# Tzq2doc/distributed_learning_simulator

Hardware: AMD Instinct MI355X
Metric: FL rounds/sec (FedAvg, 100 clients, ResNet-18, CIFAR-10-shaped) (higher is better)
Workload: dtype fp32; 1 GPU; fedavg_resnet18; model=ResNet18, algo=fed_avg, clients=100, local_epochs=5, global_batch=6400, per_client_batch=64, parallelism=client-dp1, backend=hip

## Files before the change

csrc/conv_halo.hip:

```cpp
#include "dls.h"
#include "epilogue_f32.h"
#include "gemm_common.h"

namespace {

typedef __attribute__((address_space(3))) void lds_void;

__device__ __forceinline__ void hdma16(__amdgpu_buffer_rsrc_t r, unsigned char* lds, uint32_t off) {
  __builtin_amdgcn_raw_ptr_buffer_load_lds(r, (lds_void*)lds, 16, off, 0, 0, 0);
}

template <int N>
__device__ __forceinline__ void hwait_vm() {
  static_assert(N >= 0 && N < 64, "vmcnt range");
  __builtin_amdgcn_s_waitcnt((N & 15) | ((N >> 4) << 14) | (7 << 4) | (15 << 8));
}

template <int IMG, int TH, int TW, int BN, int WM, int WN, bool BKM, int MINW, int HB, int NBS, int BNM = 0,
          int TPS = 1>
__global__ void __launch_bounds__(WM* WN * 64) __attribute__((amdgpu_waves_per_eu(MINW * WM * WN / 4)))
conv_halo_kernel(ConvNTParams p) {
  constexpr bool BNF = BNM != 0, DENSE = BNM == 2;
  static_assert((HB == 2 && NBS == 3) || (HB == 1 && (NBS == 2 || NBS == 3)), "pipeline shape");
  static_assert(TPS == 1 || (HB == 1 && TPS == 2 && NBS == 2), "taps per step");
// ... 212 lines not shown
        const bool real = BI * NW == NBI || i * NW + wid < NBI;
        if (TPS > 1 && !real) continue;
        unsigned char* d = real ? Bs + (i * NW + wid) * 1024 : smem + SCR;
        hdma16(br, d, ok ? off : OOB_OFF);
        hdma16(br, real ? d + B_PL : d, ok ? off + b_lo : OOB_OFF);
      }
    }
  };

  f32x16 acc[TM][TN];
#pragma unroll
  for (int i = 0; i < TM; ++i)
#pragma unroll
    for (int j = 0; j < TN; ++j) acc[i][j] = f32x16{};

  const int wm0 = (wid / WN) * (TM * 32), wn0 = (wid % WN) * (TN * 32);
  const int g = lane >> 4, q = (lane >> 2) & 3, pp = lane & 3, h = lane >> 5;
  int hbase[TM], hkey[TM];
#pragma unroll
  for (int i = 0; i < TM; ++i) {
    const int pix = wm0 + i * 32 + (lane & 31);
    const int img = pix / (TH * TW), rr = pix - img * (TH * TW);
    const int th = rr / TW, tw = rr - th * TW;
    hbase[i] = img * HH2 * PITCH + th * PITCH + tw;
    hkey[i] = (img * HH2 + th) * KC;
  }
  const int rsw = (lane >> 2) & 3;
  auto compute = [&](int hb, int slot, int shift, int dh) {
    const unsigned char* Hs = smem + H_OFF + hb * 2 * H_PL;
    const unsigned char* Bs = smem + B_OFF + slot * 2 * B_PL;
#pragma unroll
    for (int ks = 0; ks < 2; ++ks) {
      bf16x8 ah[TM], al[TM], bh[TN], bl[TN];
#pragma unroll
      for (int i = 0; i < TM; ++i) {
        const int hr = hbase[i] + shift;
        const unsigned char* a = Hs + hr * 64 + (((ks * 2 + h) ^ (((hr >> 2) + hkey[i] + dh * KC) & 3)) << 4);
        ah[i] = *reinterpret_cast<const bf16x8*>(a);
        al[i] = *reinterpret_cast<const bf16x8*>(a + H_PL);
      }
#pragma unroll
      for (int j = 0; j < TN; ++j) {
        if constexpr (!BKM) {
          const unsigned char* b = Bs + (wn0 + j * 32 + (lane & 31)) * 64 + (((ks * 2 + h) ^ rsw) << 4);
          bh[j] = *reinterpret_cast<const bf16x8*>(b);
          bl[j] = *reinterpret_cast<const bf16x8*>(b + B_PL);
        } else {
          const int kr = ks * 16 + 8 * h + q;
          const int f = SS > 1 ? (kr / SD) & (SS - 1) : 0;
          const int col = (wn0 + j * 32 + 16 * (g & 1) + 4 * pp) ^ (f << 5);
          const bf16_t* b0p = reinterpret_cast<const bf16_t*>(Bs) + kr * BN + col;
          bh[j] = tr_frag(b0p, b0p + 4 * BN);
          bl[j] = tr_frag(b0p + B_PL / 2, b0p + B_PL / 2 + 4 * BN);
        }
      }
#pragma unroll
      for (int i = 0; i < TM; ++i)
#pragma unroll
        for (int j = 0; j < TN; ++j) {
          acc[i][j] = __builtin_amdgcn_mfma_f32_32x32x16_bf16(al[i], bh[j], acc[i][j], 0, 0, 0);
          acc[i][j] = __builtin_amdgcn_mfma_f32_32x32x16_bf16(ah[i], bl[j], acc[i][j], 0, 0, 0);
          acc[i][j] = __builtin_amdgcn_mfma_f32_32x32x16_bf16(ah[i], bh[j], acc[i][j], 0, 0, 0);
        }
    }
  };

  if constexpr (COEF_C > 0) {
    for (int i = threadIdx.x; i < 2 * p.C; i += NW * 64) coef_s[i] = bcoef[i];
    __syncthreads();
  }
  issue_halo(0, 0);
  issue_w(0, 0);
  if constexpr (NBS == 3) issue_w(1, 1);
  if constexpr (TPS > 1) {
    int c = 0, j = 0;
    for (int s = 0; s < nsteps; ++s) {
      if (j == 0 && c > 0) {
        __builtin_amdgcn_s_barrier();
        issue_halo(c, 0);
        hwait_vm<0>();
      } else {
        hwait_vm<TPS * GB*(NBS - 2)>();
      }
      __builtin_amdgcn_s_barrier();
      issue_w(s + NBS - 1, (s + NBS - 1) % NBS);
#pragma unroll
      for (int u = 0; u < TPS; ++u) {
        const int tap = j * TPS + u;
        if (tap < 9) {
          const int dh = tap / 3;
          compute(0, (s % NBS) * TPS + u, dh * PITCH + (tap - dh * 3), dh);
        }
      }
      if (++j == SPC) {
        j = 0;
        ++c;
      }
    }
  } else {
  int c = 0, tap = 0;
  for (int s = 0; s < nsteps; ++s) {
    if constexpr (HB == 2) {
      if (tap == 1 || tap == 2)
        hwait_vm<GB + GH>();
      else
        hwait_vm<GB>();
    } else {
      if (tap == 0 && c > 0) {
        __builtin_amdgcn_s_barrier();
        issue_halo(c, 0);
        hwait_vm<0>();
      } else {
        hwait_vm<GB*(NBS - 2)>();
      }
    }
    __builtin_amdgcn_s_barrier();
    issue_w(s + NBS - 1, (s + NBS - 1) % NBS);
    if constexpr (HB == 2)
      if (tap == 0) issue_halo(c + 1, (c + 1) & 1);
    const int dh = tap / 3;
    compute(HB == 2 ? (c & 1) : 0, s % NBS, dh * PITCH + (tap - dh * 3), dh);
    if (++tap == 9) {
      tap = 0;
      ++c;
    }
  }
  }
  hwait_vm<0>();

  nt_f32_epilogue<TM, TN, NW, (TM * TN <= 2 ? 2 : -1), false>(p, acc, smem, client, m0, n0, wm0, wn0, wid, lane);
}

template <int IMG, int TH, int TW, int BN, int WM, int WN, int HB, int NBS, int TPS = 1, int MINW = 1>
void launch_halo(const ConvNTParams& p, int K, hipStream_t s) {
  const int tilesM = IMG == 1 ? p.B * (p.OH / TH) : p.B / IMG;
  const int grid = K * tilesM * cdiv(p.N, BN);
  if (p.b_kmajor)
    hipLaunchKernelGGL((conv_halo_kernel<IMG, TH, TW, BN, WM, WN, true, MINW, HB, NBS, 0, TPS>), dim3(grid),
                       dim3(WM * WN * 64), 0, s, p);
  else
    hipLaunchKernelGGL((conv_halo_kernel<IMG, TH, TW, BN, WM, WN, false, MINW, HB, NBS, 0, TPS>), dim3(grid),
                       dim3(WM * WN * 64), 0, s, p);
}

template <int IMG, int TH, int TW, int BN, int WM, int WN, int NBS, int BNM = 1, int TPS = 1, int MINW = 1>
void launch_halo_bnf(const ConvNTParams& p, int K, hipStream_t s) {
  const int tilesM = IMG == 1 ? p.B * (p.OH / TH) : p.B / IMG;
  const int grid = K * tilesM * cdiv(p.N, BN);
  hipLaunchKernelGGL((conv_halo_kernel<IMG, TH, TW, BN, WM, WN, false, MINW, 1, NBS, BNM, TPS>), dim3(grid),
                     dim3(WM * WN * 64), 0, s, p);
}


int g_halo_mode = -1;
int g_halo_variant = -1;

}

void conv_halo_set_mode(int m) { g_halo_mode = m; }
void conv_halo_set_variant(int v) { g_halo_variant = v; }

static int halo_config(const ConvNTParams& p) {
  if (p.KH != 3 || p.KW != 3 || p.stride != 1 || p.pad != 1 || p.pad_w != 1 || p.dil != 1) return -1;
  const bool dense = p.bn_x != nullptr && p.bn_c > 0;
  if (p.OH != p.H || p.OW != p.W || p.out_s > 1 || p.C % 32 || p.N % (dense ? 4 : 8) || p.ldx % 8 || p.R != 9 * p.C)
    return -1;
  if ((p.x_lo == 0 && p.bn_x == nullptr) || p.wsplit == nullptr) return -1;
  if (p.bn_x != nullptr && (p.b_kmajor || (!dense && p.ldx != p.C))) return -1;
  if (p.bn_x != nullptr && p.C > (dense ? (p.OW == 8 ? 1 << 30 : 512) : (p.OW == 32 ? 128 : p.OW == 8 ? 256 : 1 << 30)))
    return -1;
  if (dense) {
    if (p.N > 32 || p.bn_c % 4 || p.bn_c > p.C || p.bn_c > p.ldx || (p.bn_y && p.bn_ldy % 4)) return -1;
    if (p.bn_mask && (!p.bn_y || p.bn_ldy % 8 || p.bn_c % 8)) return -1;
    if (p.OW == 32 && p.OH % 8 == 0) return 4;
    if (p.OW == 16 && p.OH == 16) return 5;
    if (p.OW == 8 && p.OH == 8 && p.B % 4 == 0) return 6;
    return -1;
  }
  if (p.OW == 32 && p.OH % 8 == 0 && p.N <= 64) return 0;
  if (p.OW == 16 && p.OH == 16) return 1;
  if (p.OW == 8 && p.OH == 8 && p.B % 2 == 0) return 2;
  if (p.OW == 4 && p.OH == 4 && p.B % 8 == 0 && g_halo_mode == 1) return 3;
  return -1;
}

bool conv_halo(const ConvNTParams& p, int K, hipStream_t s) {
  if (g_halo_mode == 0 || p.yp) return false;
  const int cfg = halo_config(p);
  if (cfg < 0) return false;
  const long ab = (p.x_lo + (long)p.B * p.H * p.W * p.ldx) * 2;
  const long wb = (p.ws_plane + (p.b_kmajor ? (long)p.C * p.wKH * p.wKW * p.N : (long)p.N * p.R)) * 2;
  if (ab >= (long)OOB_OFF || wb >= (long)OOB_OFF) return false;
  if (p.bn_x != nullptr) {
    if (g_halo_variant >= 0 || cfg == 3) return false;
    switch (cfg) {
      case 0: launch_halo_bnf<1, 8, 32, 64, 4, 2, 2, 1, 2, 2>(p, K, s); break;
      case 1: launch_halo_bnf<1, 16, 16, 128, 4, 2, 2>(p, K, s); break;
      case 2: launch_halo_bnf<2, 8, 8, 128, 4, 2, 2>(p, K, s); break;
      case 4: launch_halo_bnf<1, 8, 32, 32, 4, 1, 3, 2>(p, K, s); break;
      case 5: launch_halo_bnf<1, 16, 16, 32, 4, 1, 3, 2>(p, K, s); break;
      case 6: launch_halo_bnf<4, 8, 8, 32, 4, 1, 3, 2>(p, K, s); break;
      default: return false;
    }
    return true;
  }
  const int v = g_halo_variant >= 0 ? g_halo_variant : (cfg == 2 ? 2 : 1);
  if (cfg > 3) return false;
  if (cfg == 0 && (v == 1 || v == 3)) {
    launch_halo<1, 8, 32, 64, 4, 2, 1, 2, 2>(p, K, s);
    return true;
  }
  if (v > 2) return false;
  switch (cfg * 3 + v) {
    case 0: launch_halo<1, 8, 32, 64, 4, 1, 2, 3>(p, K, s); break;
    case 2: launch_halo<1, 8, 32, 64, 4, 2, 2, 3>(p, K, s); break;
    case 3: launch_halo<1, 16, 16, 128, 4, 2, 2, 3>(p, K, s); break;
    case 4: launch_halo<1, 16, 16, 128, 4, 2, 1, 2>(p, K, s); break;
    case 5: launch_halo<1, 16, 16, 128, 4, 2, 1, 3>(p, K, s); break;
    case 6: launch_halo<2, 8, 8, 128, 2, 2, 2, 3>(p, K, s); break;
    case 7: launch_halo<2, 8, 8, 128, 4, 2, 1, 3>(p, K, s); break;
    case 8: launch_halo<2, 8, 8, 128, 4, 2, 1, 2>(p, K, s); break;
    case 9: launch_halo<8, 4, 4, 128, 2, 2, 2, 3>(p, K, s); break;
    case 10: launch_halo<8, 4, 4, 128, 4, 2, 1, 3>(p, K, s); break;
    case 11: launch_halo<8, 4, 4, 128, 4, 2, 1, 2>(p, K, s); break;
    default: return false;
  }
  return true;
}

bool conv_halo_bn_supported(int B, int H, int W, int C, int N) {
  ConvNTParams p{};
  p.bn_x = reinterpret_cast<const float*>(16);
  p.wsplit = reinterpret_cast<const bf16_t*>(16);
  p.B = B; p.H = H; p.W = W; p.C = C; p.OH = H; p.OW = W; p.KH = 3; p.KW = 3;
  p.stride = 1; p.pad = 1; p.pad_w = 1; p.dil = 1; p.N = N; p.R = 9 * C; p.ldx = C; p.out_s = 1;
  const int cfg = halo_config(p);
  return g_halo_mode != 0 && g_halo_variant < 0 && cfg >= 0 && cfg != 3 && (long)B * H * W * C * 4 < (1L << 31);
}

static ConvNTParams halo_bn_params(const float* x, long x_cs, int ldx, const float* coef, int relu,
                                   const int* valid_rows, const bf16_t* wsplit, long ws_cs, long ws_plane, int rep,
                                   float* y, long y_cs, int ldy, int B, int H, int W, int C, int N, float* stats,
                                   const int* stats_valid) {
  ConvNTParams p{};
  p.f32 = 1;
  p.bn_x = x;
  p.bn_x_cs = x_cs;
  p.bn_coef = coef;
  p.bn_relu = relu;
  p.bn_valid = valid_rows;
  p.wsplit = wsplit;
  p.ws_cs = ws_cs;
  p.ws_plane = ws_plane;
  p.rep = rep;
  p.y = reinterpret_cast<bf16_t*>(y);
  p.y_cs = y_cs;
  p.B = B; p.H = H; p.W = W; p.C = C; p.OH = H; p.OW = W; p.KH = 3; p.KW = 3;
  p.stride = 1; p.pad = 1; p.pad_w = 1; p.dil = 1;
  p.M = B * H * W; p.N = N; p.R = 9 * C;
  p.wKH = 3; p.wKW = 3; p.kh_off = 2; p.kw_off = 2; p.kh_step = 1; p.kw_step = 1;
  p.out_s = 1;
  p.ldx = ldx; p.ldy = ldy;
  p.fd_ohw = make_fastdiv((uint32_t)(H * W));
  p.fd_ow = make_fastdiv((uint32_t)W);
  p.fd_kwc = make_fastdiv((uint32_t)(3 * C));
  p.fd_c = make_fastdiv((uint32_t)C);
  p.stats = stats;
  p.stats_valid = stats_valid;
  return p;
}

bool conv_halo_bn_fwd(const float* x, long x_cs, const float* coef, int relu, const int* valid_rows,
                      const bf16_t* wsplit, long ws_cs, long ws_plane, int rep, float* y, long y_cs, int K, int B,
                      int H, int W, int C, int N, float* stats, const int* stats_valid, hipStream_t s,
                      bf16_t* yp, uint8_t* mask) {
  ConvNTParams p = halo_bn_params(x, x_cs, C, coef, relu, valid_rows, wsplit, ws_cs, ws_plane, rep, y, y_cs, N, B, H,
                                  W, C, N, stats, stats_valid);
  p.bn_yp = yp;
  p.bn_mask = mask;
  if (stats && stats_valid && !yp && native_option(g_opt_halo_skip, "DLS_SKIP_INVALID", 1)) {
    p.skip_valid = stats_valid;
    p.skip_mul = H * W;
  }
  const long wb = (ws_plane + (long)N * p.R) * 2;
  if (wb >= (long)OOB_OFF || (long)p.M * C * 4 >= (1L << 31)) return false;
  return conv_halo(p, K, s);
}

bool conv_halo_bn_dense_supported(int B, int H, int W, int C, int N) {
  ConvNTParams p{};
  p.bn_x = reinterpret_cast<const float*>(16);
  p.wsplit = reinterpret_cast<const bf16_t*>(16);
  p.bn_c = 4;
  p.B = B; p.H = H; p.W = W; p.C = C; p.OH = H; p.OW = W; p.KH = 3; p.KW = 3;
  p.stride = 1; p.pad = 1; p.pad_w = 1; p.dil = 1; p.N = N; p.R = 9 * C; p.ldx = C; p.out_s = 1;
  return g_halo_mode != 0 && g_halo_variant < 0 && halo_config(p) >= 4;
}

bool conv_halo_bn_dense_fwd(const float* x, long x_cs, int ldx, int creal, const float* coef, int relu,
                            const int* valid_rows, const bf16_t* wsplit, long ws_cs, long ws_plane, int rep, float* y,
                            long y_cs, int ldy, int K, int B, int H, int W, int C, int N, float* stats,
                            const int* stats_valid, float* ny, long ny_cs, int ldny, uint8_t* mask, hipStream_t s) {
  ConvNTParams p = halo_bn_params(x, x_cs, ldx, coef, relu, valid_rows, wsplit, ws_cs, ws_plane, rep, y, y_cs, ldy, B,
                                  H, W, C, N, stats, stats_valid);
  p.bn_c = creal;
  p.bn_y = ny;
  p.bn_y_cs = ny_cs;
  p.bn_ldy = ldny;
  p.bn_mask = mask;
  const long wb = (ws_plane + (long)N * p.R) * 2;
  if (wb >= (long)OOB_OFF || (long)p.M * ldx * 4 >= (1L << 31)) return false;
  if (halo_config(p) < 4) return false;
  return conv_halo(p, K, s);
}
```

csrc/dls.h:

```cpp
#pragma once
#include <hip/hip_runtime.h>
#include <stdint.h>

typedef uint16_t bf16_t;

constexpr int kOptUnset = -1000000;
extern int g_opt_attn_mfma, g_opt_conv_gl, g_opt_pl_min_wg;
extern int g_opt_halo_wgrad_unroll;
extern int g_opt_halo_skip;
extern int g_opt_conv_pix;
int native_option(int& slot, const char* env, int dflt);
bool set_native_option(const char* name, int value);

struct FastDiv {
  uint32_t d, mul, shift;
};

static inline FastDiv make_fastdiv(uint32_t d) {
  FastDiv f;
  f.d = d;
  uint32_t s = 0;
  while ((1u << s) < d) ++s;
  f.shift = s;
  f.mul = (uint32_t)((((uint64_t)1 << 32) * (((uint64_t)1 << s) - d)) / d + 1);
  return f;
}

__device__ __forceinline__ uint32_t fdiv(uint32_t n, const FastDiv& f) {
  return (__umulhi(n, f.mul) + n) >> f.shift;
}

struct ConvNTParams {
  const bf16_t* x;
  const bf16_t* w;
  bf16_t* y;
  const bf16_t* bias;
  const bf16_t* acc;
  long acc_cs;
  int acc_compact;
  const uint8_t* acc_mask;
  const bf16_t* gate;
  long x_cs, y_cs, w_cs, b_cs;
  int B, H, W, C;
  int OH, OW, KH, KW, stride, pad, dil;
  int pad_w;
  int M, N, R;
  int rep;
  int relu;
  int b_kmajor;
  int wKH, wKW, kh_off, kh_step, kw_off, kw_step;
  int out_s, out_ph, out_pw, out_H, out_W;
  FastDiv fd_ohw, fd_ow, fd_kwc, fd_c;
  int f32;
  int ldx, ldy;
  float* stats;
  const int* stats_valid;
  const uint32_t* drop_seeds;
  float drop_p;
  float out_scale;
  const bf16_t* wsplit;
  long ws_cs, ws_plane;
  long x_lo;
  float* bnb;
  const float* bnb_x;
  long bnb_xld;
  const float* bnb_y;
  const uint8_t* bnb_mask;
  const float* bnb_mean;
  const float* bnb_rstd;
  const int* bnb_valid;
  const float* bn_x;
  long bn_x_cs;
  const float* bn_coef;
  int bn_relu;
  const int* bn_valid;
  bf16_t* bn_yp;
  uint8_t* bn_mask;
  int bn_c;
  float* bn_y;
  long bn_y_cs;
  int bn_ldy;
  const int* skip_valid;
  int skip_mul;
  bf16_t* yp;
  long yp_cs, yp_lo;
  int pix;
  FastDiv fd_pb;
};

struct BNBwdPartials {
  float* part;
  const float* x;
  long xld;
  const float* y;
  const uint8_t* mask;
  const float* mean;
  const float* rstd;
  const int* valid;
};

struct DenseWgradParams {
  const float* dy;
  long dy_cs;
  int ldy;
  const float* y;
  long y_cs;
  float* dw;
  long dw_cs;
  float* part;
  int K, B, H, W, C, N, nchunks, G;
  const float* bn_sc;
  int ldy_x;
  const int* valid_rows;
};

struct DenseDgradParams {
  const float* dy;
  long dy_cs;
  int ldy;
  const float* w;
  long w_cs;
  int rep;
  const float* x;
  float* dx;
  long x_cs;
  int ldx;
  const uint8_t* mask;
  const float* y;
  const float* bn_sc;
  const float* mean;
  const float* rstd;
  const int* valid_rows;
  const float* coef;
  float* part;
  int K, B, H, W, C, N, G, nchunks;
};

struct SgdEpi {
  float* theta;
  float* mom;
  bf16_t* split;
  long th_cs, sp_cs, sp_lo;
  const float* lr;
  const uint8_t* active;
  const uint8_t* first;
  float wd, momentum, dampening;
  int nesterov;
};

struct HaloWgradParams {
  const void* dy;
  long dy_cs, dy_lo;
  int ldy;
  const void* x;
  long x_cs, x_lo;
  int ldx;
  const float* coef;
  int relu;
  const int* x_valid;
  const int* valid_img;
  const float* bb_x;
  const uint8_t* bb_mask;
  const float* bb_coef;
// ... 261 lines not shown
```

csrc/elementwise.hip:

```cpp
#include <algorithm>

#include "common.h"
#include "sgd_epi.h"
#include "dls.h"
#include <cstdlib>
#include <cstring>
#include <stdexcept>

namespace {

template <typename T>
__global__ void pool_fwd_kernel(const T* __restrict__ x, T* __restrict__ y, int* __restrict__ idx,
                                long total, int H, int W, int C, int OH, int OW, int k, int stride, int pad,
                                int mode) {
  const long i = (long)blockIdx.x * blockDim.x + threadIdx.x;
  if (i >= total) return;
  const int c = i % C;
  long t = i / C;
  const int ow = t % OW;
  t /= OW;
  const int oh = t % OH;
  const long img = t / OH;
  const T* xi = x + img * H * W * C;
  float best = -INFINITY, acc = 0.f;
// ... 910 lines not shown
}

void delta_rows(const float* theta, const float* base, float* out, int K, long P, long ld, hipStream_t s) {
  dim3 grid(grid_for(P / 4, 256, 1024), K);
  hipLaunchKernelGGL(delta_kernel, grid, dim3(256), 0, s, theta, base, out, P / 4, ld);
}

void weighted_sum(const float* x, const double* w, double* out, int K, long P, long ld, hipStream_t s) {
  hipLaunchKernelGGL(weighted_sum_kernel, dim3(grid_for(P / 4, 256, 8192)), dim3(256), 0, s, x, w, out, K, P / 4, ld);
}

void mix_rows(const float* x, const float* w, void* out, int K, int M, long P, long ld, long ld_out, int f32,
              hipStream_t s) {
  if (K > MIX_KMAX || M <= 0) {
    CHECK_HIP(hipErrorInvalidValue);
    return;
  }
  dim3 grid(grid_for(P / 4, 256, 2048), cdiv(M, MIX_M));
  DISPATCH_T(f32, hipLaunchKernelGGL(mix_rows_kernel<TT>, grid, dim3(256), 0, s, x, w, MP(out), K, M, P / 4, ld,
                                     ld_out));
}

void masked_weighted_sum(const float* x, const uint8_t* mask, const double* w, double* num, double* den, int K, long P,
                         long ld, hipStream_t s) {
  hipLaunchKernelGGL(masked_weighted_sum_kernel, dim3(grid_for(P, 256, 8192)), dim3(256), 0, s, x, mask, w, num, den,
                     K, P, ld);
}

void dropout_mask(uint8_t* mask, int K, long P, float p, const uint32_t* seeds, hipStream_t s) {
  const long n = (long)K * P;
  hipLaunchKernelGGL(dropout_mask_kernel, dim3(cdiv(n, 256)), dim3(256), 0, s, mask, P, p, seeds, n);
}

void block_sq_norms(const float* x, const int* block_ids, float* out, int K, long P, long ld, int nblocks,
                    hipStream_t s) {
  CHECK_HIP(hipMemsetAsync(out, 0, sizeof(float) * K * nblocks, s));
  dim3 grid(grid_for(P / 16, 256, 1024), K);
  hipLaunchKernelGGL(block_sq_kernel, grid, dim3(256), 0, s, x, block_ids, out, P, ld, nblocks);
}

void seg_minmax(const float* x, const int* seg, float* mn, float* mx, int K, long P, long ld, int nseg,
                hipStream_t s) {
  dim3 grid(cdiv(P, 256), K);
  hipLaunchKernelGGL(seg_minmax_kernel, grid, dim3(256), 0, s, x, seg, mn, mx, P, ld, nseg);
}

void stochastic_qdq(float* x, const int* seg, const float* mn, const float* mx, int K, long P, long ld, int nseg,
                    const uint32_t* seed, int levels, hipStream_t s) {
  dim3 grid(grid_for(P, 256, 2048), K);
  hipLaunchKernelGGL(stochastic_qdq_kernel, grid, dim3(256), 0, s, x, seg, mn, mx, P, ld, nseg, seed, levels);
}

void nnadq_qdq(float* x, const int* seg, const float* lo, const float* scale, const float* levels, int K, long P,
               long ld, int nseg, hipStream_t s) {
  dim3 grid(grid_for(P, 256, 2048), K);
  hipLaunchKernelGGL(nnadq_qdq_kernel, grid, dim3(256), 0, s, x, seg, lo, scale, levels, P, ld, nseg);
}

void sign_pack(const float* g, uint8_t* out, int K, long P, long ld, hipStream_t s) {
  const long nbytes = (P + 7) / 8;
  dim3 grid(grid_for(nbytes, 256, 2048), K);
  hipLaunchKernelGGL(sign_pack_kernel, grid, dim3(256), 0, s, g, out, P, ld, nbytes);
}

void sign_vote(const uint8_t* packed, const uint8_t* active, int* votes, int K, long P, hipStream_t s) {
  hipLaunchKernelGGL(sign_vote_kernel, dim3(grid_for(P, 256, 8192)), dim3(256), 0, s, packed, active, votes, K, P,
                     (P + 7) / 8);
}

void embedding_fwd(const int* tokens, const void* table, void* out, int K, long n_tok, int D, long t_cs, int rep,
                   int f32, hipStream_t s, float scale, const float* pe, int L) {
  const long total = (long)K * n_tok * D;
  DISPATCH_T(f32, hipLaunchKernelGGL(embedding_fwd_kernel<TT>, dim3(cdiv(total, 256)), dim3(256), 0, s, tokens,
                                     CP(table), MP(out), n_tok, D, t_cs, rep, total, scale, pe, L > 0 ? L : 1));
}

void embedding_bwd(const int* tokens, const void* dy, float* dtable, int K, long n_tok, int D, long t_cs, int f32,
                   hipStream_t s, float scale) {
  const long total = (long)K * n_tok * D;
  DISPATCH_T(f32, hipLaunchKernelGGL(embedding_bwd_kernel<TT>, dim3(cdiv(total, 256)), dim3(256), 0, s, tokens, CP(dy),
                                     dtable, n_tok, D, t_cs, total, scale));
}

void embedding_bwd_sorted(const int* keys, const int* order, const void* dy, float* dtable, long n, int D, int V,
                          long t_cs, int f32, hipStream_t s, float scale, float* part) {
  if (part) {
    const long nch = cdiv(n, (long)EMB_CH);
    DISPATCH_T(f32, hipLaunchKernelGGL(embedding_bwd_chunk_kernel<TT>, dim3(cdiv(nch, 4L)), dim3(256), 0, s, keys,
                                       order, CP(dy), dtable, part, n, D, V, t_cs, scale));
    DISPATCH_T(f32, hipLaunchKernelGGL(embedding_bwd_join_kernel<TT>, dim3(cdiv(nch, 4L)), dim3(256), 0, s, keys,
                                       part, dtable, n, D, V, t_cs, scale));
    return;
  }
  DISPATCH_T(f32, hipLaunchKernelGGL(embedding_bwd_sorted_kernel<TT>, dim3(cdiv(n, 4)), dim3(256), 0, s, keys, order,
                                     CP(dy), dtable, n, D, V, t_cs, scale));
}
long embedding_bwd_part_floats(long n, int D) { return cdiv(n, (long)EMB_CH) * 2 * D; }

void seq_mean_fwd(const void* x, const int* len, void* y, long S, int L, int D, int f32, hipStream_t s) {
  const long total = S * D;
  DISPATCH_T(f32, hipLaunchKernelGGL(seq_mean_fwd_kernel<TT>, dim3(cdiv(total, 256)), dim3(256), 0, s, CP(x), len,
                                     MP(y), L, D, total));
}

void seq_mean_bwd(const void* dy, const int* len, void* dx, long S, int L, int D, int f32, hipStream_t s) {
  const long total = S * L * D;
  DISPATCH_T(f32, hipLaunchKernelGGL(seq_mean_bwd_kernel<TT>, dim3(cdiv(total, 256)), dim3(256), 0, s, CP(dy), len,
                                     MP(dx), L, D, total));
}

void gather_rows(const void* src, const int* idx, void* dst, long n, long row_bytes, hipStream_t s) {
  const long v16 = row_bytes / 16;
  hipLaunchKernelGGL(gather_rows_kernel, dim3(cdiv(n * v16, 256)), dim3(256), 0, s, static_cast<const uint4*>(src), idx,
                     static_cast<uint4*>(dst), n, v16);
}

void dropout_apply(const void* x, void* out, int K, long rows, int N, long ld, const uint32_t* seeds, float p,
                   float scale, int f32, hipStream_t s) {
  const long total = rows * (long)N;
  if (total == 0 || K == 0) return;
  const dim3 grid((unsigned)std::min<long>(cdiv(total, 256), 4096), K);
  if (f32)
    hipLaunchKernelGGL(dropout_apply_kernel<float>, grid, dim3(256), 0, s, static_cast<const float*>(x),
                       static_cast<float*>(out), rows, N, ld, seeds, p, scale);
  else
    hipLaunchKernelGGL(dropout_apply_kernel<bf16_t>, grid, dim3(256), 0, s, static_cast<const bf16_t*>(x),
                       static_cast<bf16_t*>(out), rows, N, ld, seeds, p, scale);
}

long dropout_planes_ws_floats(int K, long rows, int N) { return (long)K * cdiv(rows, DP_RB) * N; }

void dropout_planes(const float* x, float* out, bf16_t* yp, int K, long rows, int N, const uint32_t* seeds, float p,
                    float scale, hipStream_t s, float* colsum, long colsum_cs, float* ws) {
  if (rows == 0 || K == 0) return;
  if (N % 2) throw std::runtime_error("dropout_planes: N must be even");
  const dim3 grid((unsigned)cdiv(rows, DP_RB), K);
  hipLaunchKernelGGL(dropout_planes_kernel, grid, dim3(256), 0, s, x, out, yp, rows, N, seeds, p, scale,
                     colsum ? ws : nullptr);
  if (colsum) fold_col_partials(ws, (int)grid.x, N, colsum, colsum_cs, K, s);
}

void synth_images(const int64_t* idx, long n, long npix, int C, int Cout, const int* source, const float* proto,
                  unsigned long long salt, float sqrt6, float noise, float* out, hipStream_t s) {
  const long total = n * (npix / C) * Cout;
  if (total == 0) return;
  hipLaunchKernelGGL(synth_images_kernel, dim3((unsigned)std::min<long>(cdiv(total, 256), 65536)), dim3(256), 0, s,
                     idx, n, npix, C, Cout, source, proto, salt, sqrt6, noise, out);
}

int g_opt_attn_mfma = kOptUnset, g_opt_conv_gl = kOptUnset;
int g_opt_pl_min_wg = kOptUnset;
int g_opt_halo_wgrad_unroll = kOptUnset, g_opt_halo_skip = kOptUnset;
int g_opt_conv_pix = kOptUnset;

int native_option(int& slot, const char* env, int dflt) {
  if (slot == kOptUnset) {
    const char* e = getenv(env);
    slot = e ? atoi(e) : dflt;
  }
  return slot;
}

bool set_native_option(const char* name, int value) {
  struct Entry {
    const char* name;
    int* slot;
  };
  const Entry table[] = {{"attn_mfma", &g_opt_attn_mfma},
                         {"conv_gl", &g_opt_conv_gl},       {"pl_min_wg", &g_opt_pl_min_wg},
                         {"halo_wgrad_unroll", &g_opt_halo_wgrad_unroll}, {"halo_skip", &g_opt_halo_skip},
                         {"conv_pix", &g_opt_conv_pix}};
  for (const Entry& t : table)
    if (strcmp(t.name, name) == 0) {
      *t.slot = value;
      return true;
    }
  return false;
}
```

Before: 0.2966 rounds/s.

## Add pipelined 3x3 halo conv kernel for 32-wide feature maps

Adds a dedicated 512-thread halo convolution kernel for the 8x32 tile / 64-channel case. It double-buffers halo rows and weight taps (two taps per stage) and prefetches the next channel chunk into registers while MFMA work runs on the current one. The BN-fused variant applies the scale/shift, ReLU, hi/lo split and mask writes during staging. It is on by default through a new native option, and it trades register pressure and extra barriers for better overlap of memory with compute in the first ResNet stage.

```diff
diff --git a/csrc/conv_halo.hip b/csrc/conv_halo.hip
--- a/csrc/conv_halo.hip
+++ b/csrc/conv_halo.hip
@@ -388,6 +388,309 @@
 }
 
 
+template <bool BKM, bool BNF>
+__global__ void __launch_bounds__(512) __attribute__((amdgpu_waves_per_eu(4)))
+conv_halo_pipe_kernel(ConvNTParams p) {
+  constexpr int TH = 8, TW = 32, BN = 64, WN = 2, NW = 8, TM = 2, TN = 1, TPS = 2, SPC = 5;
+  constexpr int BM = TH * TW;
+  constexpr int PITCH = TW + 2, HP = (TH + 2) * PITCH;
+  constexpr int HI = (HP + 16 * NW - 1) / (16 * NW);
+  constexpr int H_PL = HI * 16 * NW * 64, B_PL = BN * 64;
+  constexpr int NBI = BN / 16;
+  constexpr int B_OFF = 2 * H_PL;
+  constexpr int LOOP = B_OFF + 2 * TPS * 2 * B_PL;
+  constexpr int EPI = NW * 32 * (TN * 32 + 4) * 4;
+  constexpr int SMEM = LOOP > EPI ? LOOP : EPI;
+  constexpr int PF = 2 * HI;
+  constexpr int COEF_OFF = HP * 64;
+  static_assert(COEF_OFF + 128 * 8 <= H_PL, "BN coefficients of 128 channels behind the halo rows");
+  __shared__ __attribute__((aligned(1024))) unsigned char smem[SMEM];
+
+  const int lane = threadIdx.x & 63;
+  const int wid = __builtin_amdgcn_readfirstlane(threadIdx.x >> 6);
+  const int tpi = p.OH / TH;
+  const int tilesM = p.B * tpi;
+  const int bid = xcd_remap(blockIdx.x, gridDim.x);
+  const int client = bid / tilesM;
+  const int tm = bid - client * tilesM, m0 = tm * BM;
+  if (p.skip_valid && m0 >= p.skip_valid[client] * p.skip_mul) {
+    const int parts = (p.M + 31) / 32;
+    for (int i = threadIdx.x; i < (BM / 32) * BN; i += NW * 64) {
+      const int g = m0 / 32 + i / BN, n = i % BN;
+      if (g < parts && n < p.N) {
+        const long o = ((long)client * parts + g) * 2 * p.N + n;
+        if (p.stats) {
+          p.stats[o] = 0.f;
+          p.stats[o + p.N] = 0.f;
+        }
+        if (p.bnb) {
+          p.bnb[o] = 0.f;
+          p.bnb[o + p.N] = 0.f;
+        }
+      }
+    }
+    return;
+  }
+  const long a_img = (long)p.B * p.H * p.W * p.ldx;
+  const auto ar = make_rsrc(p.x + (long)client * p.x_cs, (uint32_t)((p.x_lo + a_img) * 2));
+  const uint32_t a_lo = (uint32_t)(p.x_lo * 2);
+  const long w_ext = BKM ? (long)p.C * p.wKH * p.wKW * p.N : (long)p.N * p.R;
+  const auto br = make_rsrc(p.wsplit + (long)(client / p.rep) * p.ws_cs, (uint32_t)((p.ws_plane + w_ext) * 2));
+  const uint32_t b_lo = (uint32_t)(p.ws_plane * 2);
+
+  const int bn_rows = BNF ? (p.bn_valid ? p.bn_valid[client] : p.B * p.H * p.W) : 0;
+  const int nchunks = p.C / 32;
+  const float* bxc = BNF ? p.bn_x + (long)client * p.bn_x_cs : nullptr;
+  const float* bcoef = BNF ? p.bn_coef + (long)client * p.C * 2 : nullptr;
+  const long bn_rc = (long)p.B * p.H * p.W * p.C;
+  bf16_t* bn_yph = (BNF && p.bn_yp) ? p.bn_yp + (long)client * 2 * bn_rc : nullptr;
+  uint8_t* bn_mk = (BNF && p.bn_mask) ? p.bn_mask + (long)client * (bn_rc >> 3) : nullptr;
+
+  const int b0 = tm / tpi, h0 = (tm - b0 * tpi) * TH;
+  const int lc = (lane & 3) ^ ((lane >> 4) & 3);
+  int h_off[HI];
+  int h_fl[HI];
+#pragma unroll
+  for (int i = 0; i < HI; ++i) {
+    const int hr = (i * NW + wid) * 16 + (lane >> 2);
+    const int hh = hr / PITCH, ww = hr - hh * PITCH;
+    const int ih = h0 - p.pad + hh, iw = ww - p.pad_w;
+    const int pix = (b0 * p.H + ih) * p.W + iw;
+    const bool ok = hr < HP && (unsigned)ih < (unsigned)p.H && (unsigned)iw < (unsigned)p.W;
+    h_off[i] = ok ? pix * p.ldx + lc * 8 : -1;
+    if constexpr (BNF)
+      h_fl[i] = (pix < bn_rows ? 1 : 0) | (ok && hh >= 1 && hh <= TH && ww >= 1 && ww <= TW ? 2 : 0);
+  }
+  constexpr int CPR = BN / 8, RPI = 64 / CPR;
+  constexpr int SD = 128 / BN, SS = BN / 32;
+  const long wkhwn = (long)p.wKH * p.wKW * p.N;
+  const int wlc = (lane & 3) ^ ((lane >> 4) & 3);
+  int b_off;
+  if constexpr (!BKM) {
+    const int n = wid * 16 + (lane >> 2);
+    b_off = n < p.N ? n * p.R + wlc * 8 : -1;
+  } else {
+    const int kr = wid * RPI + lane / CPR;
+    const int f = (kr / SD) & (SS - 1);
+    const int n = ((lane % CPR) ^ (f << 2)) * 8;
+    b_off = n < p.N ? (int)(kr * wkhwn) + n : -1;
+  }
+
+  auto dma_halo = [&](int c) {
+#pragma unroll
+    for (int i = 0; i < HI; ++i) {
+      const bool ok = h_off[i] >= 0;
+      unsigned char* d = smem + (i * NW + wid) * 1024;
+      const uint32_t off = (uint32_t)(h_off[i] + c * 32) * 2u;
+      hdma16(ar, d, ok ? off : OOB_OFF);
+      hdma16(ar, d + H_PL, ok ? off + a_lo : OOB_OFF);
+    }
+  };
+  u32x4_t pf[PF];
+  auto prefetch = [&](int c) {
+#pragma unroll
+    for (int i = 0; i < HI; ++i) {
+      const bool ok = h_off[i] >= 0;
+      if constexpr (!BNF) {
+        const uint32_t off = (uint32_t)(h_off[i] + c * 32) * 2u;
+        pf[2 * i] = __builtin_amdgcn_raw_buffer_load_b128(ar, ok ? off : OOB_OFF, 0, 0);
+        pf[2 * i + 1] = __builtin_amdgcn_raw_buffer_load_b128(ar, ok ? off + a_lo : OOB_OFF, 0, 0);
+      } else {
+        const int e = (ok ? h_off[i] : 0) + c * 32;
+        pf[2 * i] = *reinterpret_cast<const u32x4_t*>(bxc + e);
+        pf[2 * i + 1] = *reinterpret_cast<const u32x4_t*>(bxc + e + 4);
+      }
+    }
+  };
+  const float* coef_s = reinterpret_cast<const float*>(smem + COEF_OFF);
+  auto stage = [&](int c) {
+    float4 c0, c1, c2, c3;
+    if constexpr (BNF) {
+      const float4* cf = reinterpret_cast<const float4*>(coef_s + 2 * (c * 32 + lc * 8));
+      c0 = cf[0], c1 = cf[1], c2 = cf[2], c3 = cf[3];
+    }
+#pragma unroll
+    for (int i = 0; i < HI; ++i) {
+      unsigned char* d = smem + (i * NW + wid) * 1024 + lane * 16;
+      if constexpr (!BNF) {
+        *reinterpret_cast<u32x4_t*>(d) = pf[2 * i];
+        *reinterpret_cast<u32x4_t*>(d + H_PL) = pf[2 * i + 1];
+      } else {
+        const bool ok = h_off[i] >= 0;
+        const bool okv = ok && (h_fl[i] & 1);
+        const int e = (ok ? h_off[i] : 0) + c * 32;
+        const u32x4_t x0 = pf[2 * i], x1 = pf[2 * i + 1];
+        float v[8] = {fmaf(__uint_as_float(x0.x), c0.x, c0.y), fmaf(__uint_as_float(x0.y), c0.z, c0.w),
+                      fmaf(__uint_as_float(x0.z), c1.x, c1.y), fmaf(__uint_as_float(x0.w), c1.z, c1.w),
+                      fmaf(__uint_as_float(x1.x), c2.x, c2.y), fmaf(__uint_as_float(x1.y), c2.z, c2.w),
+                      fmaf(__uint_as_float(x1.z), c3.x, c3.y), fmaf(__uint_as_float(x1.w), c3.z, c3.w)};
+#pragma unroll
+        for (int j = 0; j < 8; ++j) {
+          if (p.bn_relu) v[j] = fmaxf(v[j], 0.f);
+          if (!okv) v[j] = 0.f;
+        }
+        uint32_t hi[4], lo[4];
+#pragma unroll
+        for (int j = 0; j < 4; ++j) split_pair(v[2 * j], v[2 * j + 1], hi[j], lo[j]);
+        if ((i * NW + wid) * 16 + (lane >> 2) < HP) {
+          *reinterpret_cast<uint4*>(d) = make_uint4(hi[0], hi[1], hi[2], hi[3]);
+          *reinterpret_cast<uint4*>(d + H_PL) = make_uint4(lo[0], lo[1], lo[2], lo[3]);
+        }
+        if ((bn_yph || bn_mk) && ok && (h_fl[i] & 2)) {
+          if (bn_yph) {
+            *reinterpret_cast<uint4*>(bn_yph + e) = make_uint4(hi[0], hi[1], hi[2], hi[3]);
+            *reinterpret_cast<uint4*>(bn_yph + bn_rc + e) = make_uint4(lo[0], lo[1], lo[2], lo[3]);
+          }
+          if (bn_mk) {
+            uint32_t m = 0;
+#pragma unroll
+            for (int j = 0; j < 8; ++j) m |= (v[j] > 0.f ? 1u : 0u) << j;
+            bn_mk[e >> 3] = (uint8_t)m;
+          }
+        }
+      }
+    }
+    __builtin_amdgcn_s_waitcnt(0xC07F);
+  };
+  auto issue_w = [&](int s, int slot) {
+    if (wid >= NBI) return;
+    const int c = s / SPC, j = s - c * SPC;
+#pragma unroll
+    for (int u = 0; u < TPS; ++u) {
+      const int tap = j * TPS + u;
+      if (tap >= 9) continue;
+      int boff;
+      if constexpr (!BKM) {
+        boff = tap * p.C + c * 32;
+      } else {
+        const int kh2 = tap / 3, kw2 = tap - kh2 * 3;
+        const int khh = p.kh_off - p.kh_step * kh2, kww = p.kw_off - p.kw_step * kw2;
+        boff = (int)(c * 32 * wkhwn) + (khh * p.wKW + kww) * p.N;
+      }
+      unsigned char* d = smem + B_OFF + (slot * TPS + u) * 2 * B_PL + wid * 1024;
+      const uint32_t off = (uint32_t)(b_off + boff) * 2u;
+      hdma16(br, d, b_off >= 0 ? off : OOB_OFF);
+      hdma16(br, d + B_PL, b_off >= 0 ? off + b_lo : OOB_OFF);
+    }
+  };
+
+  f32x16 acc[TM][TN];
+  const int wm0 = (wid / WN) * (TM * 32), wn0 = (wid % WN) * (TN * 32);
+  const int g = lane >> 4, q = (lane >> 2) & 3, pp = lane & 3, h = lane >> 5;
+  int hbase[TM];
+#pragma unroll
+  for (int i = 0; i < TM; ++i) {
+    const int pix = wm0 + i * 32 + (lane & 31);
+    hbase[i] = (pix / TW) * PITCH + pix % TW;
+  }
+  const int rsw = (lane >> 2) & 3;
+  auto compute = [&](int tile, int shift) {
+    const unsigned char* Bs = smem + B_OFF + tile * 2 * B_PL;
+#pragma unroll
+    for (int ks = 0; ks < 2; ++ks) {
+      bf16x8 ah[TM], al[TM], bh[TN], bl[TN];
+#pragma unroll
+      for (int i = 0; i < TM; ++i) {
+        const int hr = hbase[i] + shift;
+        const unsigned char* a = smem + hr * 64 + (((ks * 2 + h) ^ ((hr >> 2) & 3)) << 4);
+        ah[i] = *reinterpret_cast<const bf16x8*>(a);
+        al[i] = *reinterpret_cast<const bf16x8*>(a + H_PL);
+      }
+#pragma unroll
+      for (int j = 0; j < TN; ++j) {
+        if constexpr (!BKM) {
+          const unsigned char* b = Bs + (wn0 + j * 32 + (lane & 31)) * 64 + (((ks * 2 + h) ^ rsw) << 4);
+          bh[j] = *reinterpret_cast<const bf16x8*>(b);
+          bl[j] = *reinterpret_cast<const bf16x8*>(b + B_PL);
+        } else {
+          const int kr = ks * 16 + 8 * h + q;
+          const int f = (kr / SD) & (SS - 1);
+          const int col = (wn0 + j * 32 + 16 * (g & 1) + 4 * pp) ^ (f << 5);
+          const bf16_t* b0p = reinterpret_cast<const bf16_t*>(Bs) + kr * BN + col;
+          bh[j] = tr_frag(b0p, b0p + 4 * BN);
+          bl[j] = tr_frag(b0p + B_PL / 2, b0p + B_PL / 2 + 4 * BN);
+        }
+      }
+#pragma unroll
+      for (int i = 0; i < TM; ++i)
+#pragma unroll
+        for (int j = 0; j < TN; ++j) {
+          acc[i][j] = __builtin_amdgcn_mfma_f32_32x32x16_bf16(al[i], bh[j], acc[i][j], 0, 0, 0);
+          acc[i][j] = __builtin_amdgcn_mfma_f32_32x32x16_bf16(ah[i], bl[j], acc[i][j], 0, 0, 0);
+          acc[i][j] = __builtin_amdgcn_mfma_f32_32x32x16_bf16(ah[i], bh[j], acc[i][j], 0, 0, 0);
+        }
+    }
+  };
+
+  if constexpr (BNF) {
+    prefetch(0);
+    for (int i = threadIdx.x; i < 2 * p.C; i += NW * 64) reinterpret_cast<float*>(smem + COEF_OFF)[i] = bcoef[i];
+    __syncthreads();
+  } else {
+    dma_halo(0);
+  }
+  issue_w(0, 0);
+  if constexpr (BNF) stage(0);
+#pragma unroll
+  for (int i = 0; i < TM; ++i)
+#pragma unroll
+    for (int j = 0; j < TN; ++j) acc[i][j] = f32x16{};
+  auto taps = [&](int s, int j) {
+#pragma unroll
+    for (int u = 0; u < TPS; ++u) {
+      const int tap = j * TPS + u;
+      if (tap < 9) {
+        const int dh = tap / 3;
+        compute((s & 1) * TPS + u, dh * PITCH + (tap - dh * 3));
+      }
+    }
+  };
+#pragma clang loop unroll(disable)
+  for (int c = 0; c < nchunks; ++c) {
+    const bool more = c + 1 < nchunks;
+    int s = c * SPC, j0 = 0, j1 = 1;
+    asm volatile("" : "+s"(j0), "+s"(j1));
+    hwait_vm<0>();
+    if (c > 0) {
+      __builtin_amdgcn_s_barrier();
+      stage(c);
+    }
+    __builtin_amdgcn_s_barrier();
+    issue_w(s + 1, (s + 1) & 1);
+    if (more) prefetch(c + 1);
+    taps(s, j0);
+    ++s;
+    if (more)
+      hwait_vm<PF>();
+    else
+      hwait_vm<0>();
+    __builtin_amdgcn_s_barrier();
+    issue_w(s + 1, (s + 1) & 1);
+    taps(s, j1);
+#pragma clang loop unroll(disable)
+    for (int j = 2; j < SPC; ++j) {
+      ++s;
+      hwait_vm<0>();
+      __builtin_amdgcn_s_barrier();
+      if (j + 1 < SPC || more) issue_w(s + 1, (s + 1) & 1);
+      taps(s, j);
+    }
+  }
+  hwait_vm<0>();
+  int em0 = m0;
+  asm volatile("" : "+s"(em0));
+  nt_f32_epilogue<TM, TN, NW, 2, false>(p, acc, smem, client, em0, 0, wm0, wn0, wid, lane);
+}
+
+template <bool BNF>
+void launch_halo_pipe(const ConvNTParams& p, int K, hipStream_t s) {
+  const dim3 grid(K * p.B * (p.OH / 8)), block(512);
+  if (p.b_kmajor && !BNF)
+    hipLaunchKernelGGL((conv_halo_pipe_kernel<true, false>), grid, block, 0, s, p);
+  else
+    hipLaunchKernelGGL((conv_halo_pipe_kernel<false, BNF>), grid, block, 0, s, p);
+}
+
 int g_halo_mode = -1;
 int g_halo_variant = -1;
 
@@ -395,6 +698,8 @@
 
 void conv_halo_set_mode(int m) { g_halo_mode = m; }
 void conv_halo_set_variant(int v) { g_halo_variant = v; }
+
+static bool halo_pipe_on() { return native_option(g_opt_halo_pipe, "DLS_HALO_PIPE", 1) > 0; }
 
 static int halo_config(const ConvNTParams& p) {
   if (p.KH != 3 || p.KW != 3 || p.stride != 1 || p.pad != 1 || p.pad_w != 1 || p.dil != 1) return -1;
@@ -430,7 +735,12 @@
   if (p.bn_x != nullptr) {
     if (g_halo_variant >= 0 || cfg == 3) return false;
     switch (cfg) {
-      case 0: launch_halo_bnf<1, 8, 32, 64, 4, 2, 2, 1, 2, 2>(p, K, s); break;
+      case 0:
+        if (halo_pipe_on())
+          launch_halo_pipe<true>(p, K, s);
+        else
+          launch_halo_bnf<1, 8, 32, 64, 4, 2, 2, 1, 2, 2>(p, K, s);
+        break;
       case 1: launch_halo_bnf<1, 16, 16, 128, 4, 2, 2>(p, K, s); break;
       case 2: launch_halo_bnf<2, 8, 8, 128, 4, 2, 2>(p, K, s); break;
       case 4: launch_halo_bnf<1, 8, 32, 32, 4, 1, 3, 2>(p, K, s); break;
@@ -443,7 +753,10 @@
   const int v = g_halo_variant >= 0 ? g_halo_variant : (cfg == 2 ? 2 : 1);
   if (cfg > 3) return false;
   if (cfg == 0 && (v == 1 || v == 3)) {
-    launch_halo<1, 8, 32, 64, 4, 2, 1, 2, 2>(p, K, s);
+    if (g_halo_variant < 0 && halo_pipe_on())
+      launch_halo_pipe<false>(p, K, s);
+    else
+      launch_halo<1, 8, 32, 64, 4, 2, 1, 2, 2>(p, K, s);
     return true;
   }
   if (v > 2) return false;
diff --git a/csrc/dls.h b/csrc/dls.h
--- a/csrc/dls.h
+++ b/csrc/dls.h
@@ -9,6 +9,7 @@
 extern int g_opt_halo_wgrad_unroll;
 extern int g_opt_halo_skip;
 extern int g_opt_conv_pix;
+extern int g_opt_halo_pipe;
 int native_option(int& slot, const char* env, int dflt);
 bool set_native_option(const char* name, int value);
 
diff --git a/csrc/elementwise.hip b/csrc/elementwise.hip
--- a/csrc/elementwise.hip
+++ b/csrc/elementwise.hip
@@ -1086,6 +1086,7 @@
 int g_opt_pl_min_wg = kOptUnset;
 int g_opt_halo_wgrad_unroll = kOptUnset, g_opt_halo_skip = kOptUnset;
 int g_opt_conv_pix = kOptUnset;
+int g_opt_halo_pipe = kOptUnset;
 
 int native_option(int& slot, const char* env, int dflt) {
   if (slot == kOptUnset) {
@@ -1103,7 +1104,8 @@
   const Entry table[] = {{"attn_mfma", &g_opt_attn_mfma},
                          {"conv_gl", &g_opt_conv_gl},       {"pl_min_wg", &g_opt_pl_min_wg},
                          {"halo_wgrad_unroll", &g_opt_halo_wgrad_unroll}, {"halo_skip", &g_opt_halo_skip},
-                         {"conv_pix", &g_opt_conv_pix}};
+                         {"conv_pix", &g_opt_conv_pix},
+                         {"halo_pipe", &g_opt_halo_pipe}};
   for (const Entry& t : table)
     if (strcmp(t.name, name) == 0) {
       *t.slot = value;
```

New measurement: 0.2987 rounds/s (median of 6 runs). Within noise of the previous version (+0.7%).
